# PABannier/biogpt.cpp

Measured on AMD Instinct MI355X. Metric: decode tokens/sec BioGPT Q4_0 n_ctx=1024, higher is better.
Workload: dtype int8; 1 GPU; greedy 200-token continuation of a 4-token prompt per GPU (main.cpp loop, -b 8, --top_k 1), BioGPT-base Q4_0, F32 KV cache, n_ctx=1024; 1 step = 1 continuation per rank; n_layer=24, d_model=1024, d_ff=4096, n_vocab=42384, n_predict=200, n_prompt=4, parallelism=replicas x1 (weights RCCL-broadcast once)

## Files before the change

biogpt.cpp_amd/csrc/engine.hip:

```cpp
#include <hip/hip_runtime.h>
#include <fcntl.h>
#include <sys/file.h>
#include <unistd.h>

#include <algorithm>
#include <chrono>
#include <cmath>
#include <cstdlib>
#include <functional>
#include <memory>
#include <mutex>
#include <set>
#include <string>
#include <thread>
#include <vector>

#include "host_common.h"
#include "kernels.hip.h"
#include "kernels_fast.hip.h"
#include "kernels_decode.hip.h"
#include "kernels_fdecode.hip.h"
#include "kernels_lmhead.hip.h"
#include "kernels_sweep.hip.h"
#include "kernels_xlong.hip.h"
// ... 643 lines not shown
struct ResidentArgs { int32_t tok0, n_past0; uint32_t seq0; int32_t spec0; };
bool enqueue_decode_fused(biogpt_hip_ctx *c, int t_max, int tok_src, int advance, int l0 = 0, int l1 = -1, int only = -1, int n_tok = 1, float *host_row = nullptr,
                          bool *host_row_done = nullptr, int pl = -1, const ResidentArgs *ra = nullptr) {
    (void)hipGetLastError();
    const auto &hp = c->hp;
    const int D = hp.d_model, V = hp.n_vocab, P = hp.n_positions;
    const int lm_parts = fast_lm_grid(c);
    if (lm_parts > c->pmax_cap) BG_FAIL(false, "internal: arg-max partial buffer too small (%d > %d)", lm_parts, c->pmax_cap);
    const int32_t wt = ftype_to_type(hp.ftype);
    const int q81 = (wt == T_Q4_1 || wt == T_Q5_1) ? 1 : 0;
    unsigned long long *const ts = (c->opt.dbg & 96) ? c->tstamp : nullptr;
    unsigned long long *const wall = (c->opt.dbg & 64) ? c->tstamp + 128 : nullptr;
    if (l1 < 0) l1 = hp.n_layer;
    const bool pipelined = only < 0 && l0 == 0 && l1 == hp.n_layer && tok_src != 0 && (pl < 0 ? xpipe_usable(c, t_max) : (pl == 1 && xpipe_bucket_ok(c, t_max)));
    bool lm_in_kernel = false;
    if (n_tok > 1 && !pipelined) BG_FAIL(false, "internal: multi-token launches exist on the XCD pipeline only");
    if (only == -2 && !pipelined) BG_FAIL(false, "the XCD-pipelined decode step is not available for this context");
    if (pipelined) {
        bgk::XpParams xp{};
        xp.layers = c->xp_layers; xp.n_layer = hp.n_layer; xp.gran = c->xp_gran; xp.gran_l = c->xp_gran_l; xp.ctl = c->xp_ctl; xp.err_host = c->xp_err_host;
        xp.st = c->state;
        xp.tok_emb = dev_matrix(c, c->plan.embed_tokens); xp.pos_emb = dev_matrix(c, c->plan.embed_pos);
        xp.embed_scale = sqrtf((float)D);
        xp.tok_src = tok_src; xp.as_res = c->opt.xpipe_as_res;
        xp.pmax_val = c->pmax_val; xp.pmax_idx = c->pmax_idx; xp.nparts = lm_parts;
        xp.n_positions = P; xp.n_vocab = V;
        xp.eps = 1e-5f; xp.q_scale = 1.0f / sqrtf(64.0f);
        xp.P = P; xp.t_cap = std::min(P, (t_max + 63) & ~63); xp.dual = (c->opt.xpipe_dual && c->xp_gran_l != nullptr) ? 1 : 0;
        xp.exp_tab = reinterpret_cast<const uint16_t *>(c->arena + c->plan.exp_tab);
        xp.gelu_tab = reinterpret_cast<const uint16_t *>(c->arena + c->plan.gelu_tab);
        xp.gelu_p = c->xp_gelu_p; xp.gelu_n = c->xp_gelu_n; xp.gelu_z = c->xp_gelu_z; xp.exp_n = c->xp_exp_n;
        xp.x_final = c->x;
        {
            const MatSlot &m = c->plan.lm_head;
            const bool fold = xpipe_lm_folds(c);
            xp.lm = fold ? 1 : 0;
            xp.lm_blocks = lm_parts; xp.adv = fold ? advance : 0; xp.n_tok = n_tok; xp.samp = c->xp_samp;
            xp.Wlm = dev_matrix(c, m);
            xp.lm_ln_w = dev_vec(c, c->plan.ln_w); xp.lm_ln_b = dev_vec(c, c->plan.ln_b);
            xp.logits = c->logits; xp.logits_host = fold ? host_row : nullptr; xp.pmax_out_val = c->pmax_val; xp.pmax_out_idx = c->pmax_idx;
            lm_in_kernel = fold;
            if (host_row_done) *host_row_done = fold && host_row != nullptr;
            if (ra) {
                if (!(fold && host_row && advance == 0 && tok_src == 1 && xp.t_cap <= 1024 && (xp.t_cap <= 256 || xp.gran_l != nullptr))) BG_FAIL(false, "internal: a resident launch needs the lm_head inside the pipelined launch");
                xp.resident = 1; xp.mbox = c->res_mbox; xp.mbox_seq0 = ra->seq0; xp.done_host = c->res_done;
                xp.idle_ticks = (uint32_t)std::min(10000000, std::max(1, c->opt.resident_us)) * 100u;
                xp.res_tok0 = ra->tok0; xp.res_n_past0 = ra->n_past0; xp.res_dbg = c->opt.res_dbg;
                xp.res_spec0 = ra->spec0; xp.spec_rec = c->res_spec;
                xp.logits_alt = c->logits_alt; xp.logits_host_alt = c->logits_host_alt; xp.pmax_alt_val = c->pmax_val_alt; xp.pmax_alt_idx = c->pmax_idx_alt;
                if (!xp.spec_rec || !xp.logits_alt || !xp.logits_host_alt || !xp.pmax_alt_val || !xp.pmax_alt_idx) BG_FAIL(false, "internal: a resident launch without its alternate buffers");
            } else if (n_tok > 1 && !(fold && advance == 1 && tok_src == 2)) BG_FAIL(false, "internal: a multi-token launch needs the lm_head inside the pipeline");
        }
        xp.wall = ((c->opt.dbg & 128) || (ra && (c->opt.res_dbg & 32))) ? c->tstamp : nullptr;
        const hipError_t e = (hipError_t)bg_xpipe_launch(wt, xp.t_cap, bgk::xpipe_smem_bytes(xp.gelu_p + xp.gelu_n), c->stream, &xp, sizeof(xp));
        HIP_TRY(false, e);
    }
    for (int l = l0; l < l1 && !pipelined; l++) {
        const LayerSlots &L = c->plan.layers[(size_t)l];
        bgk::DecQkvParams a{};
        a.x = c->x; a.x_out = c->x;
        a.tok_emb = dev_matrix(c, c->plan.embed_tokens); a.pos_emb = dev_matrix(c, c->plan.embed_pos);
        a.embed_scale = sqrtf((float)D);
        a.tok_src = (l == 0) ? tok_src : 0;
        a.pmax_val = c->pmax_val; a.pmax_idx = c->pmax_idx; a.nparts = lm_parts;
        a.st = c->state; a.n_positions = P; a.n_vocab = V;
        a.ln_w = dev_vec(c, L.ln0_w); a.ln_b = dev_vec(c, L.ln0_b); a.eps = 1e-5f;
        a.Wqkv = dev_matrix(c, L.qkv); a.bqkv = dev_vec(c, L.qkv_b); a.q_scale = 1.0f / sqrtf(64.0f);
        a.q_out = c->q;
        a.kcache = c->memory_k + (size_t)l * P * D; a.vcache = c->memory_v + (size_t)l * P * D; a.P = P;
        a.tstamp = ts; a.wall = wall; a.wall_slot = 5 * l;
        bgk::DecAttnParams at{};
        at.q = c->q; at.kcache = a.kcache; at.vcache = a.vcache; at.st = c->state; at.P = P;
        at.t_cap = std::min(P, (t_max + 63) & ~63);
        at.exp_tab = reinterpret_cast<const uint16_t *>(c->arena + c->plan.exp_tab);
        at.oq_q = c->aq_q[0]; at.oq_d = c->aq_d[0]; at.oq_s = c->aq_s[0]; at.att_out = nullptr; at.q81 = q81;
        at.tstamp = ts ? ts + 16 : nullptr; at.wall = wall; at.wall_slot = 5 * l + 1;
        bgk::DecOprojParams op{};
        op.Wo = dev_matrix(c, L.o); op.aq_q = c->aq_q[0]; op.aq_d = c->aq_d[0]; op.aq_s = c->aq_s[0];
        op.bias = dev_vec(c, L.o_b); op.resid = c->x; op.out = c->x1;
        op.tstamp = ts ? ts + 32 : nullptr; op.wall = wall; op.wall_slot = 5 * l + 2;
        bgk::DecFc1Params f1{};
        f1.x1 = c->x1;
        f1.ln_w = dev_vec(c, L.ln1_w); f1.ln_b = dev_vec(c, L.ln1_b); f1.eps = 1e-5f;
        f1.W1 = dev_matrix(c, L.fc1); f1.b1 = dev_vec(c, L.fc1_b);
        f1.gelu_tab = reinterpret_cast<const uint16_t *>(c->arena + c->plan.gelu_tab);
        f1.oq_q = c->aq_q[1]; f1.oq_d = c->aq_d[1]; f1.oq_s = c->aq_s[1]; f1.q81 = q81;
        f1.tstamp = ts ? ts + 48 : nullptr; f1.wall = wall; f1.wall_slot = 5 * l + 3;
        bgk::DecFc2Params f2{};
        f2.W2 = dev_matrix(c, L.fc2); f2.aq_q = c->aq_q[1]; f2.aq_d = c->aq_d[1]; f2.aq_s = c->aq_s[1];
        f2.bias = dev_vec(c, L.fc2_b); f2.resid = c->x1; f2.out = c->x;
        f2.tstamp = ts ? ts + 64 : nullptr; f2.wall = wall; f2.wall_slot = 5 * l + 4;
        f2.seq = (l == hp.n_layer - 1) ? c->seq_dev : nullptr;
        hipError_t e = hipErrorInvalidValue;
        switch (wt) {
            case T_Q4_0: e = launch_decode_layer<bgk::W_Q4_0>(c, a, at, op, f1, f2, only); break;
            case T_Q4_1: e = launch_decode_layer<bgk::W_Q4_1>(c, a, at, op, f1, f2, only); break;
            case T_Q5_0: e = launch_decode_layer<bgk::W_Q5_0>(c, a, at, op, f1, f2, only); break;
            case T_Q5_1: e = launch_decode_layer<bgk::W_Q5_1>(c, a, at, op, f1, f2, only); break;
            case T_Q8_0: e = launch_decode_layer<bgk::W_Q8_0>(c, a, at, op, f1, f2, only); break;
            default: break;
        }
        HIP_TRY(false, e);
    }
    if (lm_in_kernel) { c->lm_blocks = lm_parts; return true; }
    if (only >= 0 || only == -2 || l1 < hp.n_layer) return true;
    {
        const MatSlot &m = c->plan.lm_head;
// ... 2792 lines not shown
```

biogpt.cpp_amd/csrc/engine_xpipe.inc:

```

std::mutex g_xp_mu;
biogpt_hip_ctx *g_xp_owner[64] = {};
int g_xp_lock_fd[64] = {};
int g_xp_lock_refs[64] = {};
pid_t g_xp_lock_pid[64] = {};

bool xpipe_process_lock(biogpt_hip_ctx *c) {
    if (c->device < 0 || c->device >= 64 || !c->opt.proc_lock) return true;
    std::lock_guard<std::mutex> lk(g_xp_mu);
    int &fd1 = g_xp_lock_fd[c->device];
    if (fd1 != 0 && g_xp_lock_pid[c->device] != getpid()) {
        if (fd1 > 0) (void)close(fd1 - 1);
        fd1 = 0; g_xp_lock_refs[c->device] = 0;
    }
    if (fd1 == 0) {
        g_xp_lock_pid[c->device] = getpid();
        char bus[64] = {0};
        if (hipDeviceGetPCIBusId(bus, (int)sizeof(bus) - 1, c->device) != hipSuccess) { (void)hipGetLastError(); snprintf(bus, sizeof(bus), "device%d", c->device); }
        for (char *q = bus; *q; q++) if (!((*q >= '0' && *q <= '9') || (*q >= 'a' && *q <= 'z') || (*q >= 'A' && *q <= 'Z'))) *q = '_';
        const std::string path = std::string(access("/dev/shm", W_OK) == 0 ? "/dev/shm" : "/tmp") + "/biogpt_hip_" + bus + ".lock";
        const int fd = open(path.c_str(), O_CREAT | O_RDONLY | O_CLOEXEC | O_NOFOLLOW, 0666);
        if (fd < 0) fd1 = -1;
        else if (flock(fd, LOCK_EX | LOCK_NB) == 0) fd1 = fd + 1;
        else {
// ... 8 lines not shown
    return true;
}
void xpipe_process_unlock(biogpt_hip_ctx *c) {
    if (!c->xp_proc_ref || c->device < 0 || c->device >= 64) return;
    std::lock_guard<std::mutex> lk(g_xp_mu);
    c->xp_proc_ref = false;
    if (--g_xp_lock_refs[c->device] <= 0 && g_xp_lock_fd[c->device] > 0) {
        (void)close(g_xp_lock_fd[c->device] - 1);
        g_xp_lock_fd[c->device] = 0; g_xp_lock_refs[c->device] = 0;
    }
}
std::vector<biogpt_hip_ctx *> g_xp_plain[64];

void xpipe_release(biogpt_hip_ctx *c) {
    xpipe_process_unlock(c);
    {
        std::lock_guard<std::mutex> lk(g_xp_mu);
        if (c->device >= 0 && c->device < 64 && g_xp_owner[c->device] == c) g_xp_owner[c->device] = nullptr;
    }
    if (c->fp_layers) (void)hipFree(c->fp_layers);
    if (c->fp_gran) (void)hipFree(c->fp_gran);
    if (c->fp_ctl) (void)hipFree(c->fp_ctl);
    c->fp_layers = nullptr; c->fp_gran = nullptr; c->fp_ctl = nullptr; c->fp_state = -1;
    if (c->xp_layers) (void)hipFree(c->xp_layers);
    if (c->xp_gran) (void)hipFree(c->xp_gran);
    if (c->xp_gran_l) (void)hipFree(c->xp_gran_l);
    if (c->xc_gran) (void)hipFree(c->xc_gran);
    c->xc_gran = nullptr; c->xc_lds = 0;
    if (c->xp_hop) (void)hipFree(c->xp_hop);
    if (c->xp_ctl) (void)hipFree(c->xp_ctl);
    if (c->xp_samp) (void)hipFree(c->xp_samp);
    if (c->xp_err_host) (void)hipHostFree(c->xp_err_host);
    if (c->res_mbox) (void)hipHostFree(c->res_mbox);
    if (c->res_done) (void)hipHostFree(c->res_done);
    c->res_mbox = nullptr; c->res_done = nullptr;
    c->xp_layers = nullptr; c->xp_gran = nullptr; c->xp_gran_l = nullptr; c->xp_hop = nullptr; c->xp_ctl = nullptr; c->xp_samp = nullptr; c->xp_err_host = nullptr;
}

bool xpipe_model_ok(const biogpt_hip_ctx *c) {
    const auto &hp = c->hp;
    const int32_t wt = ftype_to_type(hp.ftype);
    return (wt == T_Q4_0 || wt == T_Q4_1 || wt == T_Q5_0 || wt == T_Q5_1 || wt == T_Q8_0) && hp.d_model == 1024 && hp.d_ff == 4096 && hp.n_head == 16 &&
           hp.n_positions >= 64 && hp.n_layer >= 1;
}

extern "C" int bg_xpipe_launch(int wt, int t_cap, size_t smem_bytes, hipStream_t st, const void *params, size_t params_bytes);
extern "C" int bg_xpipe_set_lds(int wt, size_t smem_bytes);

int xpipe_last_xcd(const biogpt_hip_ctx *c) {
    const int units = 2 * c->hp.n_layer;
    return (units - 1) & 7;
}
bool xpipe_set_lds(biogpt_hip_ctx *c) {
    const size_t sm = bgk::xpipe_smem_bytes(c->xp_gelu_p + c->xp_gelu_n);
    if (sm <= 64 * 1024) return true;
    return bg_xpipe_set_lds(ftype_to_type(c->hp.ftype), sm) == (int)hipSuccess;
}

bool xpipe_place_hops(biogpt_hip_ctx *c, std::vector<bgk::XpLayer> &tab) {
    const int nl = c->hp.n_layer, mode = c->opt.hop_place;
    const size_t region = 1024, bytes = (size_t)nl * 4 * region * 8 + 16384;
    if (hipMalloc(&c->xp_hop, bytes) != hipSuccess || hipMemset(c->xp_hop, 0, bytes) != hipSuccess) return false;
    bgk::xp_u64 *base = reinterpret_cast<bgk::xp_u64 *>((reinterpret_cast<uintptr_t>(c->xp_hop) + 16383) & ~(uintptr_t)16383);
    auto cand = [&](int l, int which, int k) { return base + ((size_t)(l * 2 + which) * 2 + k) * region; };
    std::vector<int> pick((size_t)nl * 2, 0);
    if (mode != 0) {
        std::vector<bgk::XpProbe> pr;
        for (int l = 0; l < nl; l++)
            for (int which = 0; which < 2; which++) {
                const int src = (2 * l + which) & 7;
                const int dst = (l == nl - 1 && which == 1) ? (src ^ 1) : ((src + 1) & 7);
                for (int k = 0; k < 2; k++)
                    for (int line = 0; line < 2; line++) pr.push_back({cand(l, which, k) + (line ? 512 + 130 : 2), src, dst});
            }
        bgk::XpProbe *d_pr = nullptr;
        uint32_t *d_ctl = nullptr;
        unsigned long long *d_ticks = nullptr;
        const int reps = 12;
        std::vector<unsigned long long> ticks(pr.size(), 0ull);
        uint32_t err = 1u;
        if (hipMalloc(&d_pr, pr.size() * sizeof(bgk::XpProbe)) == hipSuccess && hipMalloc(&d_ctl, 128) == hipSuccess && hipMalloc(&d_ticks, pr.size() * 8) == hipSuccess &&
            hipMemcpy(d_pr, pr.data(), pr.size() * sizeof(bgk::XpProbe), hipMemcpyHostToDevice) == hipSuccess && hipMemset(d_ctl, 0, 128) == hipSuccess &&
            hipMemset(d_ticks, 0, pr.size() * 8) == hipSuccess) {
            hipLaunchKernelGGL(bgk::xp_hop_probe_kernel, dim3(256), dim3(64), 0, c->stream, d_pr, (int)pr.size(), reps, d_ctl, d_ticks, d_ctl + 16);
            if (hipStreamSynchronize(c->stream) == hipSuccess && hipMemcpy(ticks.data(), d_ticks, pr.size() * 8, hipMemcpyDeviceToHost) == hipSuccess)
                (void)hipMemcpy(&err, d_ctl + 16, 4, hipMemcpyDeviceToHost);
        }
        (void)hipGetLastError();
        if (d_pr) (void)hipFree(d_pr);
        if (d_ctl) (void)hipFree(d_ctl);
        if (d_ticks) (void)hipFree(d_ticks);
        if (hipMemset(c->xp_hop, 0, bytes) != hipSuccess) return false;
        if (err == 0u) {
            double gain = 0.0;
            for (int r = 0; r < nl * 2; r++) {
                unsigned long long t[2];
                for (int k = 0; k < 2; k++) t[k] = std::max(ticks[(size_t)(r * 2 + k) * 2], ticks[(size_t)(r * 2 + k) * 2 + 1]);
                const int fast = t[1] < t[0] ? 1 : 0;
                pick[(size_t)r] = mode == 2 ? 1 - fast : fast;
                gain += (double)(t[1 - fast] - t[fast]) * 10.0 / (2.0 * reps);
            }
            if (c->opt.verbose > 0) fprintf(stderr, "biogpt_hip: cross-XCD hand-off regions placed by measurement: the chosen 8 KB candidates are %.0f ns per hop faster than the others (mean over %d regions)\n", gain / (nl * 2), nl * 2);
        }
    }
    for (int l = 0; l < nl; l++) { tab[(size_t)l].gx1 = cand(l, 0, pick[(size_t)l * 2]); tab[(size_t)l].gx = cand(l, 1, pick[(size_t)l * 2 + 1]); }
    return true;
}
// ... 21 lines not shown
    for (int l = 0; l < hp.n_layer; l++) {
        const LayerSlots &L = c->plan.layers[(size_t)l];
        bgk::XpLayer &y = tab[(size_t)l];
        y.ln0_w = dev_vec(c, L.ln0_w); y.ln0_b = dev_vec(c, L.ln0_b); y.ln1_w = dev_vec(c, L.ln1_w); y.ln1_b = dev_vec(c, L.ln1_b);
        y.bqkv = dev_vec(c, L.qkv_b); y.bo = dev_vec(c, L.o_b); y.b1 = dev_vec(c, L.fc1_b); y.b2 = dev_vec(c, L.fc2_b);
        y.Wqkv = dev_matrix(c, L.qkv); y.Wo = dev_matrix(c, L.o); y.W1 = dev_matrix(c, L.fc1); y.W2 = dev_matrix(c, L.fc2);
        y.kcache = c->memory_k + (size_t)l * P * D; y.vcache = c->memory_v + (size_t)l * P * D;
    }
    const size_t gbytes = (size_t)hp.n_layer * bgk::XP_G_LAYER * 8;
    const uint32_t ctl0[3] = {1u, 0u, 1u};
    if (!xpipe_place_hops(c, tab)) { (void)hipGetLastError(); xpipe_release(c); return; }
    if (hipMalloc(&c->xp_layers, tab.size() * sizeof(bgk::XpLayer)) != hipSuccess || hipMalloc(&c->xp_gran, gbytes) != hipSuccess ||
        hipMalloc(&c->xp_ctl, 64) != hipSuccess || hipHostMalloc(reinterpret_cast<void **>(&c->xp_err_host), 64, hipHostMallocDefault) != hipSuccess ||
        hipMemcpy(c->xp_layers, tab.data(), tab.size() * sizeof(bgk::XpLayer), hipMemcpyHostToDevice) != hipSuccess ||
        hipMemset(c->xp_gran, 0, gbytes) != hipSuccess || hipMemset(c->xp_ctl, 0, 64) != hipSuccess ||
        hipMemcpy(c->xp_ctl, ctl0, 12, hipMemcpyHostToDevice) != hipSuccess ||
        hipMalloc(&c->xp_samp, 2056 * 8) != hipSuccess || hipMemset(c->xp_samp, 0, 2056 * 8) != hipSuccess) {
        (void)hipGetLastError();
        xpipe_release(c);
        return;
    }
    if (hp.n_positions > 256) {
        const size_t lbytes = (size_t)hp.n_layer * bgk::XL_G_LAYER * 8;
        if (hipMalloc(&c->xp_gran_l, lbytes) != hipSuccess || hipMemset(c->xp_gran_l, 0, lbytes) != hipSuccess) {
            (void)hipGetLastError();
            if (c->xp_gran_l) (void)hipFree(c->xp_gran_l);
    if (c->xc_gran) (void)hipFree(c->xc_gran);
    c->xc_gran = nullptr; c->xc_lds = 0;
            c->xp_gran_l = nullptr;
        }
    }
    if (c->opt.xpipe_fault) {
        const uint32_t one = 1u;
        (void)hipMemcpy(c->xp_ctl + 8, &one, 4, hipMemcpyHostToDevice);
    }
    {
        std::vector<uint16_t> tg(65536);
        for (uint32_t i = 0; i < 65536; i++) tg[i] = f32_to_f16(gelu_tanh_f32(f16_to_f32((uint16_t)i)));
        int P = 0x7C01;
        while (P > 0 && tg[(size_t)P - 1] == (uint16_t)(P - 1)) P--;
        const uint16_t Z = tg[0xFBFF];
        int N = 0x7C00;
        while (N > 0 && tg[0x8000 + (size_t)N - 1] == Z) N--;
        P = (P + 7) & ~7; N = (N + 7) & ~7;
        const size_t lds_max = 160 * 1024;
        if (P <= 0x7C00 && N <= 0x7C00 && bgk::xpipe_smem_bytes(P + N) <= lds_max) { c->xp_gelu_p = P; c->xp_gelu_n = N; c->xp_gelu_z = Z; }
    }
    if (c->xp_gelu_p + c->xp_gelu_n > 0) {
        std::vector<uint16_t> te(0x7C00);
        for (uint32_t i = 0; i < 0x7C00; i++) te[i] = f32_to_f16(expf(f16_to_f32((uint16_t)(0x8000u + i))));
        int N = 0x7C00;
        while (N > 0 && te[(size_t)N - 1] == 0) N--;
        N = (N + 7) & ~7;
        if (f32_to_f16(expf(0.0f)) == 0x3C00 && N > 0 && N <= c->xp_gelu_p + c->xp_gelu_n) c->xp_exp_n = N;
    }
    if (!xpipe_set_lds(c)) { (void)hipGetLastError(); xpipe_release(c); return; }
    *c->xp_err_host = 0u;
    c->xp_state = 1;
}

bool xpipe_bucket_ok(const biogpt_hip_ctx *c, int t_max) {
    return c->opt.xpipe && c->xp_state == 1 && (t_max <= 256 || (t_max <= 1024 && c->xp_gran_l != nullptr)) && c->device >= 0 && c->device < 64;
}
bool pipeline_slot_take(biogpt_hip_ctx *c);
bool xpipe_usable(biogpt_hip_ctx *c, int t_max) {
    if (!xpipe_bucket_ok(c, t_max)) return false;
    return pipeline_slot_take(c);
}
bool pipeline_slot_take(biogpt_hip_ctx *c) {
    if (c->device < 0 || c->device >= 64) return false;
    std::lock_guard<std::mutex> lk(g_xp_mu);
    biogpt_hip_ctx *&owner = g_xp_owner[c->device];
    if (owner != nullptr && owner != c && !owner->xp_in_call && hipStreamQuery(owner->stream) == hipSuccess) owner = nullptr;
    (void)hipGetLastError();
    if (owner == nullptr) {
        auto &pg = g_xp_plain[c->device];
        for (size_t i = 0; i < pg.size();) {
            if (pg[i] == c) { i++; continue; }
            if (hipStreamQuery(pg[i]->stream) == hipSuccess) { pg[i]->plain_inflight = false; pg.erase(pg.begin() + (long)i); }
            else { (void)hipGetLastError(); return false; }
        }
        (void)hipGetLastError();
    }
    if (owner == nullptr) owner = c;
    if (owner == c) c->xp_in_call = true;
    return owner == c;
}
bool plain_graph_begin(biogpt_hip_ctx *c) {
    if (c->device < 0 || c->device >= 64) return true;
    if (c->xp_foreign && !c->opt.graph_contended) return false;
    std::lock_guard<std::mutex> lk(g_xp_mu);
    const biogpt_hip_ctx *owner = g_xp_owner[c->device];
    if (owner != nullptr && owner != c && !c->opt.graph_contended) return false;
    if (!c->plain_inflight) { c->plain_inflight = true; g_xp_plain[c->device].push_back(c); }
    return true;
}
void plain_graph_end(biogpt_hip_ctx *c) {
    if (c->device < 0 || c->device >= 64) return;
    std::lock_guard<std::mutex> lk(g_xp_mu);
    auto &pg = g_xp_plain[c->device];
    for (size_t i = 0; i < pg.size(); i++) if (pg[i] == c) { pg.erase(pg.begin() + (long)i); break; }
    c->plain_inflight = false;
}
struct XpCallScope {
    biogpt_hip_ctx *c;
    explicit XpCallScope(biogpt_hip_ctx *ctx) : c(ctx) {}
    ~XpCallScope() {
// ... 48 lines not shown
```

biogpt.cpp_amd/csrc/kernels_xpipe.hip.h:

```cpp
#pragma once

#include "kernels_decode.hip.h"

namespace bgk {

typedef unsigned long long xp_u64;
typedef float xp_v4f __attribute__((ext_vector_type(4)));
#define XP_RLX __ATOMIC_RELAXED, __HIP_MEMORY_SCOPE_AGENT
constexpr uint32_t XP_SPIN_MAX = 400000u;

struct XpLayer {
    const float *ln0_w, *ln0_b, *ln1_w, *ln1_b;
    const float *bqkv, *bo, *b1, *b2;
    DevMatrix Wqkv, Wo, W1, W2;
    float *kcache, *vcache;
    unsigned long long *gx1, *gx;
};

constexpr int XP_G_QKV = 0;
constexpr int XP_G_ATT = 3072;
constexpr int XP_G_X1 = XP_G_ATT + 320;
constexpr int XP_G_H = XP_G_X1 + 1024;
constexpr int XP_G_X = XP_G_H + 1280;
constexpr int XP_G_LAYER = XP_G_X + 1024;
// ... 246 lines not shown
    if (WT == W_Q8_0) q = *reinterpret_cast<const uint32_t *>(m.qs + blk * 32 + j);
    else q = *reinterpret_cast<const uint32_t *>(m.qs + blk * 16 + (j & 15));
    sc = TI::q81 ? reinterpret_cast<const uint32_t *>(m.sc)[blk] : (uint32_t)reinterpret_cast<const uint16_t *>(m.sc)[blk];
    qh = (WT == W_Q5_0 || WT == W_Q5_1) ? m.qh[blk] : 0u;
}
template <int WT>
__device__ __forceinline__ void xp_row4_values(uint32_t q, uint32_t sc, uint32_t qh, int t, float (&e)[4]) {
    const int j = (4 * t) & 31;
#pragma unroll
    for (int i = 0; i < 4; i++) {
        if (WT == W_Q8_0) { e[i] = __fmul_rn((float)(int8_t)((q >> (8 * i)) & 0xFFu), h2f((uint16_t)sc)); continue; }
        const uint32_t byte = (q >> (8 * i)) & 0xFFu;
        int v = (j < 16) ? (int)(byte & 0x0Fu) : (int)(byte >> 4);
        if (WT == W_Q5_0 || WT == W_Q5_1) v |= (int)((qh >> (j + i)) & 1u) << 4;
        if (WT == W_Q4_0) e[i] = __fmul_rn((float)(v - 8), h2f((uint16_t)sc));
        else if (WT == W_Q5_0) e[i] = __fmul_rn((float)(v - 16), h2f((uint16_t)sc));
        else e[i] = __fadd_rn(__fmul_rn((float)v, h2f((uint16_t)(sc & 0xFFFFu))), h2f((uint16_t)(sc >> 16)));
    }
}

__device__ __forceinline__ uint32_t xp_pack4(int8_t q) {
    const int b = (int)(uint8_t)q;
    const int b1 = __builtin_amdgcn_update_dpp(0, b, 0x101, 0xf, 0xf, true);
    const int b2 = __builtin_amdgcn_update_dpp(0, b, 0x102, 0xf, 0xf, true);
    const int b3 = __builtin_amdgcn_update_dpp(0, b, 0x103, 0xf, 0xf, true);
    return (uint32_t)b | ((uint32_t)b1 << 8) | ((uint32_t)b2 << 16) | ((uint32_t)b3 << 24);
}

constexpr int XL_G_SC = 0;
constexpr int XL_G_PV = 16 * 1024;
constexpr int XL_G_LAYER = XL_G_PV + 16 * 16 * 128;

constexpr int XP_S_X = 0;
constexpr int XP_S_X1 = XP_S_X + 4096;
constexpr int XP_S_XQ = XP_S_X1 + 4096;
constexpr int XP_S_XD = XP_S_XQ + 1024;
constexpr int XP_S_XS = XP_S_XD + 128;
constexpr int XP_S_RED = XP_S_XS + 128;
constexpr int XP_S_HQ = XP_S_RED + 64;
constexpr int XP_S_HD = XP_S_HQ + 4096;
constexpr int XP_S_HS = XP_S_HD + 512;
constexpr int XP_S_PART = XP_S_HS + 512;
constexpr int XP_S_G = XP_S_PART + 256 * DEC_PS * 4;
constexpr int XP_S_LN = XP_S_G + 512;
constexpr int XP_S_BIAS = XP_S_LN + 16384;
constexpr int XP_S_CUR = XP_S_BIAS + 1536;
constexpr int XP_S_S = XP_S_CUR + 768;
constexpr int XP_S_REDF = XP_S_S + 1024;
constexpr int XP_S_REDD = XP_S_REDF + 512;
constexpr int XP_S_PV = XP_S_REDD + 128;
constexpr int XP_S_TOTAL = XP_S_PV + 8192;
static_assert(32 * DEC_PS2 <= 256 * DEC_PS, "fc2 block terms fit the shared region");
__host__ __device__ inline size_t xpipe_smem_bytes(int gelu_entries) { return XP_S_TOTAL + (size_t)gelu_entries * 2; }

template <int WT, bool EXPAND>
__device__ __forceinline__ float xp_dot(const Unit<WT> &u, const uint32_t *xq, float xd, float xs_f, int xs_i) {
    if constexpr (EXPAND) return unit_dot_settled<WT>(u, xq, xd, xs_f, xs_i);
    else return unit_dot_quant<WT>(u, xq, xd, xs_f, xs_i);
}
template <int WT, bool EXPAND>
__device__ __forceinline__ void xp_settle(Unit<WT> &u) {
    if constexpr (EXPAND) {
        settle_unit<WT>(u);
        asm volatile("" : "+v"(u.q0.x), "+v"(u.q0.y), "+v"(u.q0.z), "+v"(u.q0.w), "+v"(u.q1.x), "+v"(u.q1.y), "+v"(u.q1.z), "+v"(u.q1.w), "+v"(u.sc));
    }
}

__device__ __forceinline__ uint32_t xp_wave_sum_u32(uint32_t v) {
    int s = (int)v;
    s += dpp_i<DPP_QUAD_XOR1>(s); s += dpp_i<DPP_QUAD_XOR2>(s); s += dpp_i<DPP_ROW_HALF_MIRROR>(s); s += dpp_i<DPP_ROW_MIRROR>(s);
    return (uint32_t)((__builtin_amdgcn_readlane(s, 0) + __builtin_amdgcn_readlane(s, 16)) + (__builtin_amdgcn_readlane(s, 32) + __builtin_amdgcn_readlane(s, 48)));
}

template <int WT, int LPK, int NW, int KCAP, int ROLE, bool SPLIT, bool RES>
__device__ __forceinline__ void xp_run(const XpParams &p, unsigned char *smem, const int xcd, const int slot, const uint32_t epoch0, const int n_past0,
                                       const int n_gen0) {
    using TI = TypeInfo<WT>;
    static_assert(TI::quant && (WT != W_Q8_0 || SPLIT), "18-30 weight units per lane must fit the register file (Q8_0: 9 registers per unit: split layers)");
    static_assert(ROLE == 0 || ROLE == 1 || (ROLE == 2 && SPLIT), "0 attention head, 1 q/k/v rows, 2 (split layers) the MLP half");
    static_assert(SPLIT || TI::q81, "the producers publish Q8_0 block sums only for Q4_1 / Q5_1 (want_sum = q81): the symmetric formats need the signed units of the split form (unit_dot_settled)");
    constexpr bool ATTN = ROLE == 0;
    constexpr bool EXPAND = SPLIT;
    constexpr bool FIRST = !SPLIT || ROLE != 2, SECOND = !SPLIT || ROLE == 2;
    static_assert(LPK == 2 || LPK == 4 || LPK == 8 || LPK == 16, "lanes per key");
    static_assert(NW == 8 || NW == 16, "waves per workgroup");
    constexpr int D = 1024, DK = 64, NT = NW * 64;
    constexpr int QS = 96 / NW, OS = 16 / NW, FS = 64 / NW, F2R = 32 / NW;
    constexpr bool DUAL = SPLIT && KCAP > 256;
    constexpr int KW = DUAL ? KCAP / 2 : KCAP;
    constexpr int HI = (DUAL && ROLE == 1) ? 1 : 0;
    static_assert(KW % NW == 0 && KW <= NW * 64 / LPK, "key capacity of the launch");
    constexpr int NF4 = 16 / LPK, NV = KW / NW;
    float *const s_x = reinterpret_cast<float *>(smem + XP_S_X);
    float *const s_x1 = reinterpret_cast<float *>(smem + XP_S_X1);
    uint32_t *const s_xq = reinterpret_cast<uint32_t *>(smem + XP_S_XQ);
    float *const s_xd = reinterpret_cast<float *>(smem + XP_S_XD);
    uint32_t *const s_xs = reinterpret_cast<uint32_t *>(smem + XP_S_XS);
    double *const s_red = reinterpret_cast<double *>(smem + XP_S_RED);
    uint32_t *const s_hq = reinterpret_cast<uint32_t *>(smem + XP_S_HQ);
    float *const s_hd = reinterpret_cast<float *>(smem + XP_S_HD);
    uint32_t *const s_hs = reinterpret_cast<uint32_t *>(smem + XP_S_HS);
    float *const s_part = reinterpret_cast<float *>(smem + XP_S_PART);
    float *const s_g = reinterpret_cast<float *>(smem + XP_S_G);
    float *const s_ln = reinterpret_cast<float *>(smem + XP_S_LN);
    float *const s_bias = reinterpret_cast<float *>(smem + XP_S_BIAS);
    float *const s_cur = reinterpret_cast<float *>(smem + XP_S_CUR);
// ... 195 lines not shown
                        const int ix = XPK(pmax_idx)[k];
                        if (v > bv || (v == bv && ix < bi)) { bv = v; bi = ix; }
                    }
    #pragma unroll
                    for (int off = 32; off > 0; off >>= 1) {
                        const float ov = __shfl_xor(bv, off, 64);
                        const int oi = __shfl_xor(bi, off, 64);
                        if (ov > bv || (ov == bv && oi < bi)) { bv = ov; bi = oi; }
                    }
                    if (lane == 0) { s_redf[wave] = bv; s_redi[wave] = bi; }
                    __syncthreads();
                    bv = s_redf[0]; bi = s_redi[0];
    #pragma unroll
                    for (int w = 1; w < NW; w++)
                        if (s_redf[w] > bv || (s_redf[w] == bv && s_redi[w] < bi)) { bv = s_redf[w]; bi = s_redi[w]; }
                    tok = bi;
                    if (tok < 0 || tok >= XPK(n_vocab)) tok = 0;
                    if (slot == 0 && tid == 0) {
                        int32_t *tokens = state_tokens(XPK(st));
                        const int g = n_gen0;
                        if (g < XPK(n_positions)) tokens[XPK(n_positions) + g] = tok;
                        tokens[0] = tok;
                    }
                } else {
                    tok = (RES && p.resident != 0) ? XPK(res_tok0) : state_tokens(XPK(st))[0];
                }
                if (slot == 0) XP_TAIL(tk, 5);
                if (worker) {
                    float e[4];
                    if (emb_fast) {
                        uint32_t tq, tsc, tqh;
                        xp_row4_request<WT>(XPK_MATRIX(tok_emb), tok, tid, tq, tsc, tqh);
                        float te[4], pe[4];
                        xp_row4_values<WT>(pq, psc, pqh, tid, pe);
                        xp_row4_values<WT>(tq, tsc, tqh, tid, te);
    #pragma unroll
                        for (int j = 0; j < 4; j++) e[j] = __fadd_rn(__fmul_rn(te[j], XPK(embed_scale)), pe[j]);
                    } else {
    #pragma unroll
                        for (int j = 0; j < 4; j++)
                            e[j] = __fadd_rn(__fmul_rn(dequant_elem(XPK_MATRIX(tok_emb), tok, 4 * tid + j), XPK(embed_scale)), dequant_elem(XPK_MATRIX(pos_emb), n_past + 2, 4 * tid + j));
                    }
                    xv = make_float4(e[0], e[1], e[2], e[3]);
                }
            } else if (wave < 4) {
                uint32_t v[4];
                xp_sweep_q<RES, 4, 256, true>(XPL(L - 1).gx + tid, true, epoch, v, p, etag);
                xv = make_float4(__uint_as_float(v[0]), __uint_as_float(v[1]), __uint_as_float(v[2]), __uint_as_float(v[3]));
            }
            if (RES && wave < 4 && lane == 0) { s_dead[wave] = (etag == 0u) ? 1u : 0u; }
            return xv;
        };
        if constexpr (FIRST) {
        constexpr bool MERGE = SPLIT && KCAP <= 128;
        if (!attn_wg && MERGE) {
            const float4 xv = layer_input();
            if (worker) reinterpret_cast<float4 *>(s_x)[tid] = xv;
            XP_WALL(0);
        }
        if (!attn_wg && !MERGE) {
            constexpr int Q0 = (KCAP <= 192) ? QS / 3 : 0;
            Unit<WT> wqkv[QS];
#pragma unroll
            for (int s = Q0; s < QS; s++) {
                const int jj = s * 2 * NW + wave * 2 + rsub;
                load_unit<WT>(wqkv[s], XPL_MATRIX(Y.Wqkv), (int64_t)((jj >> 6) * 1024 + head * 64 + (jj & 63)) * 32 + sub);
            }
#pragma unroll
            for (int s = Q0; s < QS; s++) xp_settle<WT, EXPAND>(wqkv[s]);
            const float4 xv = layer_input();
            XP_WALL(0);
            float4 lnw = xv, lnb = xv;
            if (worker) {
                reinterpret_cast<float4 *>(s_x)[tid] = xv;
                lnw = reinterpret_cast<const float4 *>(s_ln)[tid]; lnb = reinterpret_cast<const float4 *>(s_ln + 1024)[tid];
            }
            ln4_q8_1024<TI::q81, TI::q81>(xv, lnw, lnb, p.eps, s_red, s_xq, s_xd, s_xs);
            XP_WALL(6);
            uint32_t ax[8];
            const uint4 a = *reinterpret_cast<const uint4 *>(s_xq + sub * 8), b = *reinterpret_cast<const uint4 *>(s_xq + sub * 8 + 4);
            ax[0] = a.x; ax[1] = a.y; ax[2] = a.z; ax[3] = a.w; ax[4] = b.x; ax[5] = b.y; ax[6] = b.z; ax[7] = b.w;
            const float axd = s_xd[sub];
            const uint32_t axs = s_xs[sub];
            float *const part = s_part + wave * 2 * QS * DEC_PS;
#pragma unroll
            for (int s = Q0; s < QS; s++) part[(s * 2 + rsub) * DEC_PS + sub] = xp_dot<WT, EXPAND>(wqkv[s], ax, axd, __uint_as_float(axs), (int)axs);
            __builtin_amdgcn_fence(__ATOMIC_RELEASE, "wavefront");
            __builtin_amdgcn_wave_barrier();
            __builtin_amdgcn_fence(__ATOMIC_ACQUIRE, "wavefront");
            if (lane >= 2 * Q0 && lane < 2 * QS) {
                const int jj = (lane >> 1) * 2 * NW + wave * 2 + (lane & 1);
                float v = __fadd_rn(s_bias[jj], sum32_in_order(part + lane * DEC_PS));
                const int which = jj >> 6, d = jj & 63;
                if (which == 0) v = __fmul_rn(v, p.q_scale);
                xp_put_local(G + XP_G_QKV + which * 1024 + head * 64 + d, etag, __float_as_uint(v));
                if (which != 0 && (!RES || (etag != 0u && (s_dead[0] | s_dead[1] | s_dead[2] | s_dead[3]) == 0u))) {
                    float *kc_ = Y.kcache, *vc_ = Y.vcache;
                    asm volatile("" : "+s"(kc_), "+s"(vc_));
                    ((__attribute__((address_space(1))) float *)((which == 1) ? kc_ : vc_))[((size_t)head * p.P + n_past) * DK + d] = v;
                }
            }
            XP_WALL(1);
        }
        if (attn_wg) {
            float4 kr[NF4];
            float vr[NV];
            const int ksub = tid & (LPK - 1), kidx = tid / LPK;
            const int dd = tid & (DK - 1), sl = tid >> 6;
            {
                constexpr bool KV_SC1 = !MERGE;
                const float *kb = Y.kcache + (size_t)head * p.P * DK, *vb = Y.vcache + (size_t)head * p.P * DK;
                const __amdgpu_buffer_rsrc_t krs = xp_kv_rsrc(kb, p.P * DK * 4), vrs = xp_kv_rsrc(vb, p.P * DK * 4);
                if (KV_SC1 || kidx < t_cap) {
#pragma unroll
                    for (int m = 0; m < NF4; m++) kr[m] = xp_kv_load4<KV_SC1>(krs, kb, ((HI * KW + kidx) * (DK / 4) + ksub + LPK * m) * 4);
                } else {
#pragma unroll
                    for (int m = 0; m < NF4; m++) kr[m] = make_float4(0.f, 0.f, 0.f, 0.f);
                }
#pragma unroll
                for (int k = 0; k < NV; k++) {
                    const int j = HI * KW + sl + NW * k;
                    vr[k] = (KV_SC1 || j < t_cap) ? xp_kv_load1<KV_SC1>(vrs, vb, j * DK + dd) : 0.0f;
                }
            }
            if constexpr (MERGE) {
                Unit<WT> wqkv[QS];
#pragma unroll
                for (int s = 0; s < QS; s++) {
                    const int jj = s * 2 * NW + wave * 2 + rsub;
                    load_unit<WT>(wqkv[s], XPL_MATRIX(Y.Wqkv), (int64_t)((jj >> 6) * 1024 + head * 64 + (jj & 63)) * 32 + sub);
                }
#pragma unroll
                for (int s = 0; s < QS; s++) xp_settle<WT, EXPAND>(wqkv[s]);
                const float4 xv = layer_input();
                XP_WALL(0);
                if (L == 0 && slot == 0) { asm volatile("" :: "v"(xv.x)); XP_TAIL(tk, 6); }
                float4 lnw = xv, lnb = xv;
                if (worker) {
                    reinterpret_cast<float4 *>(s_x)[tid] = xv;
                    lnw = reinterpret_cast<const float4 *>(s_ln)[tid]; lnb = reinterpret_cast<const float4 *>(s_ln + 1024)[tid];
                }
                ln4_q8_1024<TI::q81, TI::q81>(xv, lnw, lnb, p.eps, s_red, s_xq, s_xd, s_xs);
                XP_WALL(6);
                if (L == 0 && slot == 0) XP_TAIL(tk, 7);
                uint32_t ax[8];
                const uint4 a = *reinterpret_cast<const uint4 *>(s_xq + sub * 8), b = *reinterpret_cast<const uint4 *>(s_xq + sub * 8 + 4);
                ax[0] = a.x; ax[1] = a.y; ax[2] = a.z; ax[3] = a.w; ax[4] = b.x; ax[5] = b.y; ax[6] = b.z; ax[7] = b.w;
                const float axd = s_xd[sub];
                const uint32_t axs = s_xs[sub];
                float *const part = s_part + wave * 2 * QS * DEC_PS;
#pragma unroll
                for (int s = 0; s < QS; s++) part[(s * 2 + rsub) * DEC_PS + sub] = xp_dot<WT, EXPAND>(wqkv[s], ax, axd, __uint_as_float(axs), (int)axs);
                __builtin_amdgcn_fence(__ATOMIC_RELEASE, "wavefront");
                __builtin_amdgcn_wave_barrier();
                __builtin_amdgcn_fence(__ATOMIC_ACQUIRE, "wavefront");
                if (lane < 2 * QS) {
                    const int jj = (lane >> 1) * 2 * NW + wave * 2 + (lane & 1);
                    float v = __fadd_rn(s_bias[jj], sum32_in_order(part + lane * DEC_PS));
                    const int which = jj >> 6, d = jj & 63;
                    if (which == 0) v = __fmul_rn(v, p.q_scale);
                    s_cur[jj] = v;
                    if (which != 0 && (!RES || (etag != 0u && (s_dead[0] | s_dead[1] | s_dead[2] | s_dead[3]) == 0u))) {
                        float *kc_ = Y.kcache, *vc_ = Y.vcache;
                        asm volatile("" : "+s"(kc_), "+s"(vc_));
                        ((__attribute__((address_space(1))) float *)((which == 1) ? kc_ : vc_))[((size_t)head * p.P + n_past) * DK + d] = v;
                    }
                }
                XP_WALL(1);
            } else if constexpr (DUAL) {
                constexpr int QH = QS / 2;
                Unit<WT> wq[QH];
#pragma unroll
                for (int s = 0; s < QH; s++) {
// ... 185 lines not shown
                bool valid = jg < T && ksub == 0;
                if constexpr (DUAL) {
                    static_assert(LPK == 2, "two lanes per key: the second one takes the partner's score of the same index");
                    xp_u64 *const gsc = p.gran_l + (size_t)L * XL_G_LAYER + XL_G_SC + head * 1024;
                    if (valid) xp_put_local(gsc + jg, etag, __float_as_uint(sc));
                    const int jo = (1 - HI) * KW + kidx;
                    const bool theirs = ksub == 1 && jo < T;
                    uint32_t v[1];
                    xp_sweep_q<RES, 1>(gsc + jo, theirs, epoch, v, p, etag);
                    if (theirs) { sc = __uint_as_float(v[0]); valid = true; }
                }
                float mx = wave_max_f32(sc);
                if (lane == 0) s_redf[wave] = mx;
                if (RES && DUAL && lane == 0) reinterpret_cast<uint32_t *>(s_redf)[NW + wave] = (etag == 0u) ? 1u : 0u;
                __syncthreads();
                mx = s_redf[0];
#pragma unroll
                for (int w = 1; w < NW; w++) mx = fmaxf(mx, s_redf[w]);
                if constexpr (RES && DUAL) {
                    uint32_t dead = 0u;
#pragma unroll
                    for (int w = 0; w < NW; w++) dead |= reinterpret_cast<const uint32_t *>(s_redf)[NW + w];
                    if ((dead) != 0u) etag = 0u;
                }
                XP_WALL(13);
                double sum = 0.0;
                if (valid) {
                    const uint32_t ix = f2h(__fsub_rn(sc, mx)), neg = ix - 0x8000u;
                    uint16_t e16;
                    if (neg < (uint32_t)p.exp_n) e16 = s_gelu[neg];
                    else if (p.exp_n > 0 && ix == 0u) e16 = 0x3C00;
                    else if (p.exp_n > 0 && neg < 0x7C00u) e16 = 0;
                    else e16 = p.exp_tab[ix];
                    const float val = h2f(e16);
                    if (ksub == 0) s_S[kidx] = val;
                    sum = (double)val;
                }
                sum = wave_sum_f64(sum);
                if (lane == 0) s_redd[wave] = sum;
                __syncthreads();
                sum = 0.0;
#pragma unroll
                for (int w = 0; w < NW; w++) sum += s_redd[w];
                inv = inv_sum_f32(sum);
            }
            XP_WALL(14);
            {
                const float vcur = s_cur[128 + dd];
                [[maybe_unused]] const int wave_u = __builtin_amdgcn_readfirstlane(wave);
                constexpr int CH = NV < 16 ? NV : (NV % 16 == 0 ? 16 : 8);
                double a0 = 0.0, a1 = 0.0;
#pragma unroll
                for (int k0 = 0; k0 < NV; k0 += CH) {
                    float pj[CH];
#pragma unroll
                    for (int k = 0; k < CH; k++) {
                        if constexpr (SMW) pj[k] = __int_as_float(__builtin_amdgcn_readlane(__float_as_int(ev[(k0 + k) >> 3]), wave_u + 8 * ((k0 + k) & 7)));
                        else pj[k] = s_S[sl + NW * (k0 + k)];
                    }
#pragma unroll
                    for (int k = 0; k < CH; k += 2) {
                        const int j0 = HI * KW + sl + NW * (k0 + k), j1 = j0 + NW;
                        const double c0 = (double)__fmul_rn(j0 == n_past ? vcur : vr[k0 + k], __fmul_rn(pj[k], inv));
                        const double c1 = (double)__fmul_rn(j1 == n_past ? vcur : vr[k0 + k + 1], __fmul_rn(pj[k + 1], inv));
                        a0 += (j0 < T) ? c0 : 0.0;
                        a1 += (j1 < T) ? c1 : 0.0;
                    }
                }
                s_pv[tid] = a0 + a1;
            }
            __syncthreads();
            XP_WALL(15);
            if (tid < DK) {
                double t0 = 0.0, t1 = 0.0;
#pragma unroll
                for (int s2 = 0; s2 < NW; s2 += 2) { t0 += s_pv[s2 * DK + tid]; t1 += s_pv[(s2 + 1) * DK + tid]; }
                double tot = t0 + t1;
                [[maybe_unused]] xp_u64 *const gpv = DUAL ? p.gran_l + (size_t)L * XL_G_LAYER + XL_G_PV + head * 16 * 128 : nullptr;
                if constexpr (DUAL && HI == 1) {
                    xp_put_local(gpv + tid, etag, (uint32_t)__double2loint(tot)); xp_put_local(gpv + 64 + tid, etag, (uint32_t)__double2hiint(tot));
                } else {
                    if constexpr (DUAL) {
                        uint32_t v[2];
                        xp_sweep_q<RES, 2, 64>(gpv + tid, true, epoch, v, p, etag);
                        tot += __hiloint2double((int)v[1], (int)v[0]);
                    }
                    const float o = (float)tot;
                    int8_t q8; float d8; uint32_t s8;
                    q8_block32(o, TI::q81, q8, d8, s8, TI::q81);
                    const uint32_t packed = xp_pack4(q8);
                    const int blk = head * 2 + (tid >> 5);
                    if ((tid & 3) == 0) xp_put_local(G + XP_G_ATT + head * 16 + (tid >> 2), etag, packed);
                    if ((tid & 31) == 0) { xp_put_local(G + XP_G_ATT + 256 + blk, etag, __float_as_uint(d8)); if (TI::q81) xp_put_local(G + XP_G_ATT + 288 + blk, etag, s8); }
                }
            }
        }
        XP_WALL(2);
        if (wave < 5) {
            uint32_t v[1];
            xp_sweep_q<RES, 1, 1, false>(G + XP_G_ATT + tid, TI::q81 || tid < 288, epoch, v, p, etag);
            if (tid < 256) s_xq[tid] = v[0];
            else if (tid < 288) s_xd[tid - 256] = __uint_as_float(v[0]);
            else s_xs[tid - 288] = v[0];
        }
        __syncthreads();
        XP_WALL(8);
        {
            uint32_t ax[8];
            const uint4 a = *reinterpret_cast<const uint4 *>(s_xq + sub * 8), b = *reinterpret_cast<const uint4 *>(s_xq + sub * 8 + 4);
            ax[0] = a.x; ax[1] = a.y; ax[2] = a.z; ax[3] = a.w; ax[4] = b.x; ax[5] = b.y; ax[6] = b.z; ax[7] = b.w;
            const float axd = s_xd[sub];
            const uint32_t axs = s_xs[sub];
            float *const part = s_part + wave * 2 * OS * DEC_PS;
#pragma unroll
            for (int s = 0; s < OS; s++) part[(s * 2 + rsub) * DEC_PS + sub] = xp_dot<WT, EXPAND>(wo[s], ax, axd, __uint_as_float(axs), (int)axs);
            __builtin_amdgcn_fence(__ATOMIC_RELEASE, "wavefront");
            __builtin_amdgcn_wave_barrier();
// ... 352 lines not shown
```

Baseline: 4175 tokens/s.

## Extend merged QKV-attention path to longer KV caps by spilling V tail to LDS

Lets the merged QKV+attention path run for KV caps up to 256 instead of 128. It does this by staging the upper part of the prefetched V values in LDS, in an extra region placed after the exp table and in s_x1, rather than in registers. A new launch-size function reserves this extra LDS, and the exp table is only enabled when the total stays under 160KB. The aim is to keep the early V prefetch and merged schedule at longer contexts, at the cost of more LDS use and LDS reads in the PV loop.

```diff
diff --git a/biogpt.cpp_amd/csrc/engine.hip b/biogpt.cpp_amd/csrc/engine.hip
--- a/biogpt.cpp_amd/csrc/engine.hip
+++ b/biogpt.cpp_amd/csrc/engine.hip
@@ -719,7 +719,7 @@
             } else if (n_tok > 1 && !(fold && advance == 1 && tok_src == 2)) BG_FAIL(false, "internal: a multi-token launch needs the lm_head inside the pipeline");
         }
         xp.wall = ((c->opt.dbg & 128) || (ra && (c->opt.res_dbg & 32))) ? c->tstamp : nullptr;
-        const hipError_t e = (hipError_t)bg_xpipe_launch(wt, xp.t_cap, bgk::xpipe_smem_bytes(xp.gelu_p + xp.gelu_n), c->stream, &xp, sizeof(xp));
+        const hipError_t e = (hipError_t)bg_xpipe_launch(wt, xp.t_cap, bgk::xpipe_launch_smem_bytes(xp.gelu_p + xp.gelu_n, xp.exp_n), c->stream, &xp, sizeof(xp));
         HIP_TRY(false, e);
     }
     for (int l = l0; l < l1 && !pipelined; l++) {
diff --git a/biogpt.cpp_amd/csrc/engine_xpipe.inc b/biogpt.cpp_amd/csrc/engine_xpipe.inc
--- a/biogpt.cpp_amd/csrc/engine_xpipe.inc
+++ b/biogpt.cpp_amd/csrc/engine_xpipe.inc
@@ -84,7 +84,7 @@
     return (units - 1) & 7;
 }
 bool xpipe_set_lds(biogpt_hip_ctx *c) {
-    const size_t sm = bgk::xpipe_smem_bytes(c->xp_gelu_p + c->xp_gelu_n);
+    const size_t sm = bgk::xpipe_launch_smem_bytes(c->xp_gelu_p + c->xp_gelu_n, c->xp_exp_n);
     if (sm <= 64 * 1024) return true;
     return bg_xpipe_set_lds(ftype_to_type(c->hp.ftype), sm) == (int)hipSuccess;
 }
@@ -212,7 +212,7 @@
         int N = 0x7C00;
         while (N > 0 && te[(size_t)N - 1] == 0) N--;
         N = (N + 7) & ~7;
-        if (f32_to_f16(expf(0.0f)) == 0x3C00 && N > 0 && N <= c->xp_gelu_p + c->xp_gelu_n) c->xp_exp_n = N;
+        if (f32_to_f16(expf(0.0f)) == 0x3C00 && N > 0 && N <= c->xp_gelu_p + c->xp_gelu_n && bgk::xpipe_launch_smem_bytes(c->xp_gelu_p + c->xp_gelu_n, N) <= 160 * 1024) c->xp_exp_n = N;
     }
     if (!xpipe_set_lds(c)) { (void)hipGetLastError(); xpipe_release(c); return; }
     *c->xp_err_host = 0u;
diff --git a/biogpt.cpp_amd/csrc/kernels_xpipe.hip.h b/biogpt.cpp_amd/csrc/kernels_xpipe.hip.h
--- a/biogpt.cpp_amd/csrc/kernels_xpipe.hip.h
+++ b/biogpt.cpp_amd/csrc/kernels_xpipe.hip.h
@@ -322,6 +322,18 @@
 constexpr int XP_S_TOTAL = XP_S_PV + 8192;
 static_assert(32 * DEC_PS2 <= 256 * DEC_PS, "fc2 block terms fit the shared region");
 __host__ __device__ inline size_t xpipe_smem_bytes(int gelu_entries) { return XP_S_TOTAL + (size_t)gelu_entries * 2; }
+constexpr int XP_VL_FROM = 64, XP_VL_TAIL = 22, XP_VL_BYTES = XP_VL_TAIL * 512 * 4;
+static_assert((256 - XP_VL_FROM) / 8 - XP_VL_TAIL <= 2, "the slices beyond the tail fit s_x1");
+__host__ __device__ inline size_t xpipe_launch_smem_bytes(int gelu_entries, int exp_n) {
+    const size_t g = (size_t)gelu_entries * 2, a = (size_t)exp_n * 2 + XP_VL_BYTES;
+    return XP_S_TOTAL + (g > a ? g : a);
+}
+template <int WT, int KCAP, bool RES>
+__host__ __device__ constexpr bool xp_merge_fits() {
+    if (KCAP <= 128) return true;
+    if (RES || WT == W_Q8_0) return false;
+    return KCAP <= 192 || WT != W_Q4_1;
+}
 
 template <int WT, bool EXPAND>
 __device__ __forceinline__ float xp_dot(const Unit<WT> &u, const uint32_t *xq, float xd, float xs_f, int xs_i) {
@@ -623,7 +635,10 @@
             return xv;
         };
         if constexpr (FIRST) {
-        constexpr bool MERGE = SPLIT && KCAP <= 128;
+        constexpr bool MERGE = SPLIT && KCAP <= 256 && xp_merge_fits<WT, KCAP, RES>();
+        constexpr int NVL = (MERGE && KCAP > 128) ? NV - XP_VL_FROM / NW : 0, NVR = NV - NVL;
+        float *const s_vl = reinterpret_cast<float *>(smem + XP_S_TOTAL + (size_t)p.exp_n * 2) + tid, *const s_vl1 = s_x1 + tid;
+#define XP_VL(k) ((k) < XP_VL_TAIL ? s_vl + (k) * NT : s_vl1 + ((k) - XP_VL_TAIL) * NT)
         if (!attn_wg && MERGE) {
             const float4 xv = layer_input();
             if (worker) reinterpret_cast<float4 *>(s_x)[tid] = xv;
@@ -675,13 +690,24 @@
         }
         if (attn_wg) {
             float4 kr[NF4];
-            float vr[NV];
+            float vr[NVR];
             const int ksub = tid & (LPK - 1), kidx = tid / LPK;
             const int dd = tid & (DK - 1), sl = tid >> 6;
             {
                 constexpr bool KV_SC1 = !MERGE;
                 const float *kb = Y.kcache + (size_t)head * p.P * DK, *vb = Y.vcache + (size_t)head * p.P * DK;
                 const __amdgpu_buffer_rsrc_t krs = xp_kv_rsrc(kb, p.P * DK * 4), vrs = xp_kv_rsrc(vb, p.P * DK * 4);
+                if constexpr (NVL > 0) {
+                    float t[NVL];
+#pragma unroll
+                    for (int k = 0; k < NVL; k++) {
+                        const int j = sl + NW * (NVR + k);
+                        t[k] = (j < t_cap) ? xp_kv_load1<false>(vrs, vb, j * DK + dd) : 0.0f;
+                    }
+#pragma unroll
+                    for (int k = 0; k < NVL; k++) *XP_VL(k) = t[k];
+                    asm volatile("" ::: "memory");
+                }
                 if (KV_SC1 || kidx < t_cap) {
 #pragma unroll
                     for (int m = 0; m < NF4; m++) kr[m] = xp_kv_load4<KV_SC1>(krs, kb, ((HI * KW + kidx) * (DK / 4) + ksub + LPK * m) * 4);
@@ -690,7 +716,7 @@
                     for (int m = 0; m < NF4; m++) kr[m] = make_float4(0.f, 0.f, 0.f, 0.f);
                 }
 #pragma unroll
-                for (int k = 0; k < NV; k++) {
+                for (int k = 0; k < NVR; k++) {
                     const int j = HI * KW + sl + NW * k;
                     vr[k] = (KV_SC1 || j < t_cap) ? xp_kv_load1<KV_SC1>(vrs, vb, j * DK + dd) : 0.0f;
                 }
@@ -982,17 +1008,18 @@
                 double a0 = 0.0, a1 = 0.0;
 #pragma unroll
                 for (int k0 = 0; k0 < NV; k0 += CH) {
-                    float pj[CH];
+                    float pj[CH], vj[CH];
 #pragma unroll
                     for (int k = 0; k < CH; k++) {
                         if constexpr (SMW) pj[k] = __int_as_float(__builtin_amdgcn_readlane(__float_as_int(ev[(k0 + k) >> 3]), wave_u + 8 * ((k0 + k) & 7)));
                         else pj[k] = s_S[sl + NW * (k0 + k)];
+                        vj[k] = (k0 + k < NVR) ? vr[k0 + k < NVR ? k0 + k : 0] : *XP_VL(k0 + k - NVR);
                     }
 #pragma unroll
                     for (int k = 0; k < CH; k += 2) {
                         const int j0 = HI * KW + sl + NW * (k0 + k), j1 = j0 + NW;
-                        const double c0 = (double)__fmul_rn(j0 == n_past ? vcur : vr[k0 + k], __fmul_rn(pj[k], inv));
-                        const double c1 = (double)__fmul_rn(j1 == n_past ? vcur : vr[k0 + k + 1], __fmul_rn(pj[k + 1], inv));
+                        const double c0 = (double)__fmul_rn(j0 == n_past ? vcur : vj[k], __fmul_rn(pj[k], inv));
+                        const double c1 = (double)__fmul_rn(j1 == n_past ? vcur : vj[k + 1], __fmul_rn(pj[k + 1], inv));
                         a0 += (j0 < T) ? c0 : 0.0;
                         a1 += (j1 < T) ? c1 : 0.0;
                     }
```

Measured after the change: 4068 tokens/s. 2.6% lower.
